# zjkang/Relation-DETR

Hardware: AMD Instinct MI355X
Metric: images/sec @ 800×1333, 300 queries, R50 4-level; achieved HBM GB/s (higher is better)
Workload: dtype bf16; 1 GPU; relation_detr_resnet50_800_1333 transformer stack from feature pyramids: 6 encoder layers (MSDA self-attn, S=22323, 4 levels) + two-stage top-k + 6 decoder layers (relation-biased self-attn + MSDA cross-attn + box refinement) + top-300 detections; backbone/neck excluded; batch_per_gpu=4, global_batch=4, queries=900, levels=4, launch=hipGraph replay, streams=2, gemm_tuning=False, parallelism=image-parallel x1

## Files before the change

### include/relation_detr_amd.h

```cpp
#ifndef RELATION_DETR_AMD_H
#define RELATION_DETR_AMD_H

#include <stdint.h>

#ifdef __cplusplus
extern "C" {
#endif

#define RDETR_ABI_VERSION 3

typedef enum rdetr_status {
    RDETR_OK = 0,
    RDETR_ERR_INVALID_ARG = -1,
    RDETR_ERR_UNSUPPORTED = -2,
    RDETR_ERR_LAUNCH = -3
} rdetr_status;

int rdetr_abi_version(void);
const char *rdetr_status_string(int status);

int rdetr_msda_forward_f32(const float *value, const int64_t *spatial_shapes, const int64_t *level_start_index,
                           const float *sampling_loc, const float *attn_weight, int B, int S, int H, int D,
                           int L, int Nq, int P, float *out, void *stream);

// ... 144 lines not shown
int rdetr_add_layernorm_strided_f32(const float *x, const float *residual, const float *gamma, const float *beta,
                                    long long rows, int C, long long ldx, long long ldr, long long ldo, float eps,
                                    float *out, void *stream);
int rdetr_add_layernorm_strided_bf16(const uint16_t *x, const uint16_t *residual, const uint16_t *gamma,
                                     const uint16_t *beta, long long rows, int C, long long ldx, long long ldr,
                                     long long ldo, float eps, uint16_t *out, void *stream);

int rdetr_add_layernorm_pos_f32(const float *x, const float *residual, const float *gamma, const float *beta,
                                const float *pos, long long rows, int C, long long ldx, long long ldr, long long ldo,
                                long long ldp, long long ldo2, float eps, float *out, float *out2, void *stream);
int rdetr_add_layernorm_pos_bf16(const uint16_t *x, const uint16_t *residual, const uint16_t *gamma,
                                 const uint16_t *beta, const uint16_t *pos, long long rows, int C, long long ldx,
                                 long long ldr, long long ldo, long long ldp, long long ldo2, float eps, uint16_t *out,
                                 uint16_t *out2, void *stream);

int rdetr_box_refine_f32(const void *delta, int delta_is_bf16, const float *ref, long long n, float eps, float *out,
                         void *stream);
int rdetr_sine_pos_embed(const float *pos, long long rows, int n, int F, float temperature, float scale, void *out,
                         int out_is_bf16, void *stream);

int rdetr_zero_masked_rows(void *x, const unsigned char *mask, long long rows, int row_bytes, long long ld_bytes,
                           void *stream);
int rdetr_row_max(const void *x, int is_bf16, long long rows, int C, long long ldx, void *out, void *stream);

long long rdetr_topk_workspace_bytes(int rows, int n, int k);
int rdetr_topk(const void *x, int is_bf16, int rows, int n, int k, void *workspace, float *values, long long *indices, void *stream);

int rdetr_box_head_k256_bf16(const uint16_t *xa, long long lda, const uint16_t *xb, long long ldb, const uint16_t *pw1,
                             const uint16_t *b1, const uint16_t *pw2, const uint16_t *b2, const uint16_t *w3, const uint16_t *b3,
                             const float *reference, int reference_is_logit, float eps, long long M, float *out_a, float *out_b,
                             void *stream);

int rdetr_query_pos_k256_bf16(const uint16_t *emb, long long lde, const uint16_t *query, long long ldq, const uint16_t *pw1a,
                              const uint16_t *pw1b, const uint16_t *b1, const uint16_t *pw2, const uint16_t *b2, const uint16_t *pv1,
                              const uint16_t *c1, const uint16_t *pv2, const uint16_t *c2, long long M, uint16_t *out_pos,
                              uint16_t *out_qpp, void *stream);

int rdetr_encoder_proj_k256_bf16(const uint16_t *x, long long ldx, const uint16_t *xq, long long ldq, const uint16_t *pwv,
                                 const uint16_t *bv, const uint16_t *pwq, const uint16_t *bq, const uint8_t *row_mask, int B, int S,
                                 int q_cols, uint16_t *out_hm, uint16_t *out_q, void *stream);

int rdetr_detections_from_topk(const float *score, const long long *index, const float *boxes, const long long *image_sizes, int B,
                               int N, int C, int K, float *out, void *stream);

int rdetr_scaled_pos(const void *a, const void *scale, const void *query, long long n, int is_bf16, void *pos, void *qp, void *stream);

int rdetr_decoder_reference(const float *reference, const float *valid_ratios, int B, int N, int L, int F, float temperature,
                            float scale, float *ref_in, void *emb, int emb_is_bf16, void *stream);

int rdetr_pyramid_points(const unsigned char *const *level_masks, const int *level_hw, int L, int B, const unsigned char *pad_mask,
                         int keep_is_bf16, float *valid_ratios, float *reference, float *logit, void *keep, void *stream);
int rdetr_nchw_to_tokens(const void *src, const void *add_vec, int is_bf16, int B, int C, int P,
                         long long out_image_stride, long long ld_out, void *out, void *stream);

int rdetr_linear_k256_bf16(const uint16_t *x, long long ldx, const uint16_t *w, const uint16_t *bias, long long M, int N,
                           int relu, uint16_t *out, long long ldo, void *stream);

int rdetr_linear_pack_k256_bf16(const uint16_t *w, uint16_t *packed, void *stream);
int rdetr_linear_ln_k256_bf16(const uint16_t *x, long long ldx, const uint16_t *packed, const uint16_t *bias,
                              const uint16_t *residual, long long ldr, const uint16_t *gamma, const uint16_t *beta, float eps,
                              long long M, uint16_t *out, long long ldo, void *stream);

int rdetr_ffn_k256_pack_bf16(const uint16_t *w1, const uint16_t *w2, int F, uint16_t *packed, void *stream);
int rdetr_ffn_k256_bf16(const uint16_t *x, long long ldx, const uint16_t *packed, const uint16_t *b1, const uint16_t *b2,
                        long long M, int F, uint16_t *out, long long ldo, void *stream);
int rdetr_ffn_ln_k256_bf16(const uint16_t *x, long long ldx, const uint16_t *packed, const uint16_t *b1, const uint16_t *b2,
                           const uint16_t *gamma, const uint16_t *beta, float eps, const uint16_t *pos, long long ldp,
                           long long M, int F, uint16_t *out, long long ldo, uint16_t *out2, long long ldo2, void *stream);
int rdetr_ffn_k256_train_bf16(const uint16_t *x, long long ldx, const uint16_t *packed, const uint16_t *b1, const uint16_t *b2,
                              long long M, int F, uint16_t *out, long long ldo, uint16_t *hid, long long ldh, void *stream);
int rdetr_ffn_k256_backward_bf16(const uint16_t *dy, long long lddy, const uint16_t *packed_t, const uint16_t *hid, long long ldh,
                                 long long M, int F, uint16_t *dh, long long ldd, uint16_t *dx, long long lddx, void *stream);

#ifdef __cplusplus
}
#endif
#endif
```

### relation_detr_amd/_lib.py

```python
from __future__ import annotations

import ctypes
import os

_HERE = os.path.dirname(os.path.abspath(__file__))
LIB_PATH = os.environ.get("RDETR_LIB_PATH") or os.path.join(_HERE, "librelation_detr_amd.so")

_c_int, _c_float, _vp, _c_ll = ctypes.c_int, ctypes.c_float, ctypes.c_void_p, ctypes.c_longlong

SIGNATURES = {
    "rdetr_abi_version": [],
    "rdetr_status_string": [_c_int],
    "rdetr_msda_fast_path": [_c_int] * 4,
    "rdetr_msda_levels_window_ok": [_vp, _vp, _c_int, _c_ll],
    "rdetr_msda_forward_f32": [_vp] * 5 + [_c_int] * 7 + [_vp, _vp],
    "rdetr_msda_forward_bf16": [_vp] * 5 + [_c_int] * 7 + [_vp, _vp],
    "rdetr_msda_forward_fused_f32": [_vp] * 6 + [_c_int] * 8 + [_vp, _vp],
    "rdetr_msda_forward_fused_bf16": [_vp] * 6 + [_c_int] * 8 + [_vp, _vp],
    "rdetr_msda_forward_fused_ex_f32": [_vp] * 4 + [_c_int, _vp, _c_int, _vp, _c_int, _vp] + [_c_int] * 7 + [_vp, _vp],
    "rdetr_msda_forward_fused_ex_bf16": [_vp] * 4 + [_c_int, _vp, _c_int, _vp, _c_int, _vp] + [_c_int] * 7 + [_vp, _vp],
    "rdetr_msda_forward_opt_bf16": [_vp, _c_int] + [_vp] * 4 + [_c_int] * 8 + [_vp, _vp],
    "rdetr_msda_forward_sweep_bf16": [_vp, _c_int] + [_vp] * 4 + [_c_int] * 7 + [_vp, _vp],
    "rdetr_msda_forward_resident_bf16": [_vp] * 5 + [_c_int] * 7 + [_vp, _vp],
    "rdetr_msda_forward_fused_resident_bf16": [_vp, _vp, _vp, _vp, _c_int, _vp, _c_int, _vp, _c_int] + [_c_int] * 7 + [_vp, _vp],
    "rdetr_msda_forward_fused_opt_bf16": [_vp, _c_int, _vp, _vp, _vp, _c_int, _vp, _c_int, _vp, _c_int, _vp] + [_c_int] * 8 + [_vp, _vp],
    "rdetr_msda_forward_fused_strided_bf16": [_vp, _c_ll, _vp, _vp, _vp, _c_int, _vp, _c_int, _vp, _c_int, _vp] + [_c_int] * 7 + [_vp, _vp],
    "rdetr_value_to_head_major_bf16": [_vp, _c_ll, _vp] + [_c_int] * 4 + [_vp, _vp],
    "rdetr_msda_backward_f32": [_vp] * 6 + [_c_int] * 7 + [_vp] * 4,
    "rdetr_msda_backward_det_workspace_bytes": [_c_int] * 7,
    "rdetr_msda_backward_det_f32": [_vp] * 6 + [_c_int] * 7 + [_vp, _c_ll] + [_vp] * 4,
    "rdetr_msda_backward_fused_f32": [_vp] * 6 + [_c_int, _vp] + [_c_int] * 7 + [_vp, _c_ll] + [_vp] * 5,
    "rdetr_msda_backward_fused_bf16": [_vp] * 6 + [_c_int, _vp] + [_c_int] * 7 + [_vp, _c_ll] + [_vp] * 5,
    "rdetr_relation_bias_f32": [_vp] * 4 + [_c_int] * 5 + [_c_float] * 3 + [_vp, _vp],
    "rdetr_relation_bias_ws_f32": [_vp] * 4 + [_c_int] * 5 + [_c_float] * 3 + [_vp, _vp, _vp],
    "rdetr_relation_bias_backward_workspace_bytes": [_c_int] * 3,
    "rdetr_relation_bias_backward_f32": [_vp] * 4 + [_c_int] * 5 + [_c_float] * 3 + [_vp] * 4,
    "rdetr_bias_softmax_f32": [_vp] * 3 + [_c_int] * 3 + [_vp],
    "rdetr_relation_attention_bf16": [_vp] * 3 + [_c_int] * 3 + [_vp, _vp] + [_c_int] * 5 + [_c_float, _vp, _c_int, _vp],
    "rdetr_relation_attention_train_bf16": [_vp] * 3 + [_c_int] * 3 + [_vp, _vp] + [_c_int] * 5 + [_c_float, _vp, _c_int, _vp, _vp],
    "rdetr_relation_attention_backward_workspace_bytes": [_c_int] * 3,
    "rdetr_relation_attention_backward_bf16": [_vp] * 3 + [_c_int] * 3 + [_vp, _c_int, _vp, _vp, _c_int, _vp, _vp] + [_c_int] * 5
                                              + [_c_float, _vp, _c_ll] + [_vp, _c_int] * 3 + [_vp, _vp],
    "rdetr_relation_attention_boxes_bf16": [_vp] * 3 + [_c_int] * 3 + [_vp] * 5 + [_c_int] * 6 + [_c_float] * 4 + [_vp, _c_int, _vp],
    "rdetr_relation_attention_boxes_train_bf16": [_vp] * 3 + [_c_int] * 3 + [_vp] * 5 + [_c_int] * 6 + [_c_float] * 4
                                                 + [_vp, _c_int, _vp, _vp],
    "rdetr_relation_attention_boxes_backward_workspace_bytes": [_c_int] * 4,
    "rdetr_relation_attention_boxes_backward_bf16": [_vp] * 3 + [_c_int] * 3 + [_vp, _c_int, _vp, _vp, _c_int] + [_vp] * 5 + [_c_int] * 6
                                                    + [_c_float] * 4 + [_vp, _c_ll] + [_vp, _c_int] * 3 + [_vp, _vp, _vp],
    "rdetr_box_refine_f32": [_vp, _c_int, _vp, _c_ll, _c_float, _vp, _vp],
    "rdetr_sine_pos_embed": [_vp, _c_ll, _c_int, _c_int, _c_float, _c_float, _vp, _c_int, _vp],
    "rdetr_zero_masked_rows": [_vp, _vp, _c_ll, _c_int, _c_ll, _vp],
    "rdetr_row_max": [_vp, _c_int, _c_ll, _c_int, _c_ll, _vp, _vp],
    "rdetr_topk_workspace_bytes": [_c_int, _c_int, _c_int],
    "rdetr_topk": [_vp, _c_int, _c_int, _c_int, _c_int, _vp, _vp, _vp, _vp],
    "rdetr_box_head_k256_bf16": [_vp, _c_ll, _vp, _c_ll, _vp, _vp, _vp, _vp, _vp, _vp, _vp, _c_int, _c_float, _c_ll, _vp, _vp, _vp],
    "rdetr_query_pos_k256_bf16": [_vp, _c_ll, _vp, _c_ll] + [_vp] * 9 + [_c_ll, _vp, _vp, _vp],
    "rdetr_encoder_proj_k256_bf16": [_vp, _c_ll, _vp, _c_ll] + [_vp] * 5 + [_c_int, _c_int, _c_int, _vp, _vp, _vp],
    "rdetr_detections_from_topk": [_vp, _vp, _vp, _vp, _c_int, _c_int, _c_int, _c_int, _vp, _vp],
    "rdetr_scaled_pos": [_vp, _vp, _vp, _c_ll, _c_int, _vp, _vp, _vp],
    "rdetr_decoder_reference": [_vp, _vp, _c_int, _c_int, _c_int, _c_int, _c_float, _c_float, _vp, _vp, _c_int, _vp],
    "rdetr_pyramid_points": [_vp, _vp, _c_int, _c_int, _vp, _c_int, _vp, _vp, _vp, _vp, _vp],
    "rdetr_linear_k256_bf16": [_vp, _c_ll, _vp, _vp, _c_ll, _c_int, _c_int, _vp, _c_ll, _vp],
    "rdetr_linear_k256_hm_bf16": [_vp, _c_ll, _vp, _vp, _vp, _c_int, _c_int, _vp, _vp],
    "rdetr_linear_pack_k256_bf16": [_vp, _vp, _vp],
    "rdetr_linear_ln_k256_bf16": [_vp, _c_ll, _vp, _vp, _vp, _c_ll, _vp, _vp, _c_float, _c_ll, _vp, _c_ll, _vp],
    "rdetr_ffn_k256_pack_bf16": [_vp, _vp, _c_int, _vp, _vp],
    "rdetr_ffn_k256_bf16": [_vp, _c_ll, _vp, _vp, _vp, _c_ll, _c_int, _vp, _c_ll, _vp],
    "rdetr_ffn_ln_k256_bf16": [_vp, _c_ll, _vp, _vp, _vp, _vp, _vp, _c_float, _vp, _c_ll, _c_ll, _c_int, _vp, _c_ll, _vp, _c_ll, _vp],
    "rdetr_ffn_k256_train_bf16": [_vp, _c_ll, _vp, _vp, _vp, _c_ll, _c_int, _vp, _c_ll, _vp, _c_ll, _vp],
    "rdetr_ffn_k256_backward_bf16": [_vp, _c_ll, _vp, _vp, _c_ll, _c_ll, _c_int, _vp, _c_ll, _vp, _c_ll, _vp],
    "rdetr_nchw_to_tokens": [_vp, _vp, _c_int, _c_int, _c_int, _c_int, _c_ll, _c_ll, _vp, _vp],
    "rdetr_add_layernorm_f32": [_vp] * 4 + [_c_ll, _c_int, _c_float, _vp, _vp],
    "rdetr_add_layernorm_bf16": [_vp] * 4 + [_c_ll, _c_int, _c_float, _vp, _vp],
    "rdetr_add_layernorm_strided_f32": [_vp] * 4 + [_c_ll, _c_int, _c_ll, _c_ll, _c_ll, _c_float, _vp, _vp],
    "rdetr_add_layernorm_strided_bf16": [_vp] * 4 + [_c_ll, _c_int, _c_ll, _c_ll, _c_ll, _c_float, _vp, _vp],
    "rdetr_add_layernorm_pos_f32": [_vp] * 5 + [_c_ll, _c_int] + [_c_ll] * 5 + [_c_float, _vp, _vp, _vp],
    "rdetr_add_layernorm_pos_bf16": [_vp] * 5 + [_c_ll, _c_int] + [_c_ll] * 5 + [_c_float, _vp, _vp, _vp],
}

ERR_INVALID_ARG, ERR_UNSUPPORTED, ERR_LAUNCH = -1, -2, -3

_lib = None


class RdetrError(RuntimeError):
    pass


def load() -> ctypes.CDLL:
    global _lib
    if _lib is not None:
        return _lib
    if not os.path.exists(LIB_PATH):
        raise RdetrError(
            f"{LIB_PATH} not found: the HIP kernels are not built. Run `make -C relation_detr_amd/csrc` "
            "(needs hipcc, --offload-arch=gfx950). There is no CPU or PyTorch fallback for this path.")
    lib = ctypes.CDLL(LIB_PATH)
    for name, argtypes in SIGNATURES.items():
        fn = getattr(lib, name)
        fn.argtypes = argtypes
        fn.restype = ctypes.c_char_p if name == "rdetr_status_string" else (_c_ll if name.endswith("_workspace_bytes") else _c_int)
    if lib.rdetr_abi_version() != 3:
        raise RdetrError(f"ABI version mismatch: library {lib.rdetr_abi_version()}, binding 3")
    _lib = lib
    return lib


def check(status: int, what: str) -> None:
    if status != 0:
        msg = load().rdetr_status_string(status).decode()
        raise RdetrError(f"{what} failed: {msg} (status {status})")
```

### relation_detr_amd/csrc/glue.hip

```cpp
#include "common.h"

namespace rdetr {

template <typename TD> __device__ __forceinline__ float glue_load(const TD *p);
template <> __device__ __forceinline__ float glue_load<float>(const float *p) { return *p; }
template <> __device__ __forceinline__ float glue_load<uint16_t>(const uint16_t *p) { return bf16_bits_to_f32(*p); }

template <typename TD>
__global__ __launch_bounds__(256) void box_refine_kernel(const TD *__restrict__ delta, const float *__restrict__ ref, long long n,
                                                         float eps, float *__restrict__ out)
{
    const long long i = (long long)blockIdx.x * blockDim.x + threadIdx.x;
    if (i >= n) return;
    float x = ref[i];
    x = fminf(fmaxf(x, 0.f), 1.f);
    if (ref[i] != ref[i]) x = ref[i];
    const float x1 = fmaxf(x, eps), x2 = fmaxf(1.f - x, eps);
    const float z = glue_load<TD>(delta + i) + logf(x1 / x2);
    out[i] = 1.f / (1.f + expf(-z));
}

template <typename TO> __device__ __forceinline__ void glue_store(TO *p, float v);
template <> __device__ __forceinline__ void glue_store<float>(float *p, float v) { *p = v; }
template <> __device__ __forceinline__ void glue_store<uint16_t>(uint16_t *p, float v) { *p = (uint16_t)f32_to_bf16_bits(v); }
// ... 124 lines not shown
    const T *s = src + ((size_t)b * C + c0) * (size_t)P + p0;
#pragma unroll 4
    for (int i = ty; i < 64; i += 4)
        tile[i][tx] = (c0 + i < C && p0 + tx < P) ? glue_load<T>(s + (size_t)i * P + tx) : 0.f;
    __syncthreads();
    const float av = (add_vec && c0 + tx < C) ? glue_load<T>(add_vec + c0 + tx) : 0.f;
    T *o = out + (size_t)b * out_image_stride + (size_t)p0 * ld_out + c0;
#pragma unroll 4
    for (int i = ty; i < 64; i += 4)
        if (p0 + i < P && c0 + tx < C) {
            glue_store<T>(o + (size_t)i * ld_out + tx, tile[tx][i] + av);
        }
}

__global__ __launch_bounds__(256) void nchw_to_tokens_bf16_vec_kernel(const uint16_t *__restrict__ src, const uint16_t *__restrict__ add_vec,
                                                                      int C, int P, long long out_image_stride, long long ld_out,
                                                                      uint16_t *__restrict__ out)
{
    __shared__ __attribute__((aligned(16))) uint16_t tile[64][72];
    const int b = blockIdx.z, c0 = blockIdx.y * 64, p0 = blockIdx.x * 64, tid = threadIdx.x;
#pragma unroll
    for (int k = 0; k < 2; ++k) {
        const int it = tid + 256 * k, ch = it >> 3, pg = it & 7;
        u32x4 v = {0u, 0u, 0u, 0u};
        if (c0 + ch < C && p0 + 8 * pg < P)
            v = *reinterpret_cast<const u32x4 *>(src + ((size_t)b * C + c0 + ch) * (size_t)P + p0 + 8 * pg);
        const unsigned w[4] = {v.x, v.y, v.z, v.w};
#pragma unroll
        for (int j = 0; j < 4; ++j) {
            tile[8 * pg + 2 * j][ch] = (uint16_t)(w[j] & 0xffffu);
            tile[8 * pg + 2 * j + 1][ch] = (uint16_t)(w[j] >> 16);
        }
    }
    __syncthreads();
#pragma unroll
    for (int k = 0; k < 2; ++k) {
        const int it = tid + 256 * k, px = it >> 3, cg = it & 7;
        if (p0 + px >= P || c0 + 8 * cg >= C) continue;
        u32x4 v = *reinterpret_cast<const u32x4 *>(&tile[px][8 * cg]);
        if (add_vec) {
            const u32x4 a = *reinterpret_cast<const u32x4 *>(add_vec + c0 + 8 * cg);
            const unsigned vw[4] = {v.x, v.y, v.z, v.w}, aw[4] = {a.x, a.y, a.z, a.w};
            unsigned o[4];
#pragma unroll
            for (int j = 0; j < 4; ++j)
                o[j] = pack_bf16x2(bf16_bits_to_f32(vw[j] & 0xffffu) + bf16_bits_to_f32(aw[j] & 0xffffu),
                                   bf16_bits_to_f32(vw[j] >> 16) + bf16_bits_to_f32(aw[j] >> 16));
            v = u32x4{o[0], o[1], o[2], o[3]};
        }
        *reinterpret_cast<u32x4 *>(out + (size_t)b * out_image_stride + (size_t)(p0 + px) * ld_out + c0 + 8 * cg) = v;
    }
}

struct PyrLevels {
    const unsigned char *mask[8];
    int h[8], w[8], start[8];
};

__global__ __launch_bounds__(64) void valid_ratios_kernel(PyrLevels lv, int L, float *__restrict__ out)
{
    const int l = blockIdx.x, b = blockIdx.y, lane = threadIdx.x;
    const int h = lv.h[l], w = lv.w[l];
    const unsigned char *m = lv.mask[l] + (size_t)b * h * w;
    int cw = 0, ch = 0;
    for (int x = lane; x < w; x += 64) cw += m[x] == 0;
    for (int y = lane; y < h; y += 64) ch += m[(size_t)y * w] == 0;
#pragma unroll
    for (int o = 32; o >= 1; o >>= 1) {
        cw += __shfl_xor(cw, o, 64);
        ch += __shfl_xor(ch, o, 64);
    }
    if (lane == 0) {
        out[((size_t)b * L + l) * 2 + 0] = (float)cw / (float)w;
        out[((size_t)b * L + l) * 2 + 1] = (float)ch / (float)h;
    }
}

template <typename T>
__global__ __launch_bounds__(256) void pyramid_points_kernel(PyrLevels lv, int L, int S, const float *__restrict__ ratios,
                                                             const unsigned char *__restrict__ pad, float *__restrict__ reference,
                                                             float *__restrict__ logit, T *__restrict__ keep)
{
    const int s = blockIdx.x * 256 + threadIdx.x, b = blockIdx.y;
    if (s >= S) return;
    int l = 0;
    while (l + 1 < L && s >= lv.start[l + 1]) ++l;
    const int w = lv.w[l], h = lv.h[l], idx = s - lv.start[l];
    const int y = idx / w, x = idx - y * w;
    const float *vr = ratios + (size_t)b * L * 2;
    const float fx = ((float)x + 0.5f) / (vr[2 * l] * (float)w), fy = ((float)y + 0.5f) / (vr[2 * l + 1] * (float)h);
    float *r = reference + ((size_t)b * S + s) * L * 2;
    for (int k = 0; k < L; ++k) {
        r[2 * k] = fx * vr[2 * k];
        r[2 * k + 1] = fy * vr[2 * k + 1];
    }
    const float wh = 0.05f * (float)(1 << l);
    const float p[4] = {fx, fy, wh, wh};
    bool ok = !(pad && pad[(size_t)b * S + s]);
#pragma unroll
    for (int k = 0; k < 4; ++k) ok = ok && p[k] > 0.01f && p[k] < 0.99f;
    float *lg = logit + ((size_t)b * S + s) * 4;
#pragma unroll
    for (int k = 0; k < 4; ++k) lg[k] = ok ? logf(p[k] / (1.0f - p[k])) : __builtin_inff();
    glue_store<T>(keep + (size_t)b * S + s, ok ? 1.0f : 0.0f);
}

// ... 129 lines not shown
extern "C" int rdetr_zero_masked_rows(void *x, const unsigned char *mask, long long rows, int row_bytes, long long ld_bytes,
                                      void *stream)
{
    if (rows < 0 || row_bytes <= 0 || ld_bytes < row_bytes) return RDETR_ERR_INVALID_ARG;
    if ((row_bytes & 15) || (ld_bytes & 15)) return RDETR_ERR_UNSUPPORTED;
    if (rows == 0) return RDETR_OK;
    if (!x || !mask || (reinterpret_cast<uintptr_t>(x) & 15)) return RDETR_ERR_INVALID_ARG;
    const long long nblk = (rows + 255) / 256;
    if (nblk > 0x7fffffffll) return RDETR_ERR_UNSUPPORTED;
    hipLaunchKernelGGL(zero_masked_rows_kernel, dim3((unsigned)nblk), dim3(256), 0, static_cast<hipStream_t>(stream),
                       static_cast<unsigned char *>(x), mask, rows, row_bytes, ld_bytes);
    return launch_status();
}

extern "C" int rdetr_row_max(const void *x, int is_bf16, long long rows, int C, long long ldx, void *out, void *stream)
{
    if (rows < 0 || C <= 0 || ldx < C) return RDETR_ERR_INVALID_ARG;
    if (rows == 0) return RDETR_OK;
    if (!x || !out) return RDETR_ERR_INVALID_ARG;
    const long long nblk = (rows + 15) / 16;
    if (nblk > 0x7fffffffll) return RDETR_ERR_UNSUPPORTED;
    hipStream_t st = static_cast<hipStream_t>(stream);
    if (is_bf16)
        hipLaunchKernelGGL((row_max_kernel<uint16_t>), dim3((unsigned)nblk), dim3(256), 0, st, static_cast<const uint16_t *>(x), rows, C,
                           ldx, static_cast<uint16_t *>(out));
    else
        hipLaunchKernelGGL((row_max_kernel<float>), dim3((unsigned)nblk), dim3(256), 0, st, static_cast<const float *>(x), rows, C, ldx,
                           static_cast<float *>(out));
    return launch_status();
}

extern "C" int rdetr_nchw_to_tokens(const void *src, const void *add_vec, int is_bf16, int B, int C, int P,
                                    long long out_image_stride, long long ld_out, void *out, void *stream)
{
    if (B < 0 || C <= 0 || P < 0 || ld_out < C || out_image_stride < 0) return RDETR_ERR_INVALID_ARG;
    if (B == 0 || P == 0) return RDETR_OK;
    if (!src || !out) return RDETR_ERR_INVALID_ARG;
    if (B > 65535 || (C + 63) / 64 > 65535) return RDETR_ERR_UNSUPPORTED;
    const dim3 grid((unsigned)((P + 63) / 64), (unsigned)((C + 63) / 64), (unsigned)B);
    hipStream_t st = static_cast<hipStream_t>(stream);
    auto al16 = [](const void *p) { return reinterpret_cast<uintptr_t>(p) % 16 == 0; };
    if (is_bf16 && P % 8 == 0 && C % 8 == 0 && ld_out % 8 == 0 && out_image_stride % 8 == 0 && al16(src) && al16(out) &&
        (!add_vec || al16(add_vec)))
        hipLaunchKernelGGL(nchw_to_tokens_bf16_vec_kernel, grid, dim3(256), 0, st, static_cast<const uint16_t *>(src),
                           static_cast<const uint16_t *>(add_vec), C, P, out_image_stride, ld_out, static_cast<uint16_t *>(out));
    else if (is_bf16)
        hipLaunchKernelGGL((nchw_to_tokens_kernel<uint16_t>), grid, dim3(256), 0, st, static_cast<const uint16_t *>(src),
                           static_cast<const uint16_t *>(add_vec), C, P, out_image_stride, ld_out, static_cast<uint16_t *>(out));
    else
        hipLaunchKernelGGL((nchw_to_tokens_kernel<float>), grid, dim3(256), 0, st, static_cast<const float *>(src),
                           static_cast<const float *>(add_vec), C, P, out_image_stride, ld_out, static_cast<float *>(out));
    return launch_status();
}
```

### relation_detr_amd/csrc/topk.hip

```cpp
#include "common.h"

namespace rdetr {

constexpr int kTkBins = 4096;
constexpr int kTkItems = 16;
constexpr int kTkBlock = 256;
constexpr int kTkChunk = kTkBlock * kTkItems;

struct TkCtrl {
    unsigned bin, above, out_count, cand_count;
};

__device__ __forceinline__ unsigned tk_key(float v)
{
    const unsigned u = __builtin_bit_cast(unsigned, v);
    if (v != v) return 0xffffffffu;
    return (u & 0x80000000u) ? ~u : (u | 0x80000000u);
}
__device__ __forceinline__ float tk_load(const void *x, int is_bf16, size_t i)
{
    return is_bf16 ? bf16_bits_to_f32(static_cast<const uint16_t *>(x)[i]) : static_cast<const float *>(x)[i];
}
__device__ __forceinline__ float tk_value(unsigned key)
{
    if (key == 0xffffffffu) return __builtin_nanf("");
    return __builtin_bit_cast(float, (key & 0x80000000u) ? (key & 0x7fffffffu) : ~key);
}

__global__ __launch_bounds__(kTkBlock) void topk_hist_kernel(const void *__restrict__ x, int is_bf16, int n, unsigned *__restrict__ hist)
{
    __shared__ unsigned h[kTkBins];
    for (int i = threadIdx.x; i < kTkBins; i += kTkBlock) h[i] = 0;
    __syncthreads();
    const size_t row = (size_t)blockIdx.y * n;
    const int base = blockIdx.x * kTkChunk;
#pragma unroll 4
    for (int j = 0; j < kTkItems; ++j) {
        const int i = base + j * kTkBlock + threadIdx.x;
        if (i < n) atomicAdd(&h[tk_key(tk_load(x, is_bf16, row + i)) >> 20], 1u);
    }
    __syncthreads();
    unsigned *g = hist + ((size_t)blockIdx.y * gridDim.x + blockIdx.x) * kTkBins;
    for (int i = threadIdx.x; i < kTkBins; i += kTkBlock) g[i] = h[i];
}

__global__ __launch_bounds__(1024) void topk_scan_kernel(const unsigned *__restrict__ hist, int chunks, int k, TkCtrl *__restrict__ ctrl)
{
    __shared__ unsigned s[1024];
    const int t = threadIdx.x;
    unsigned c0 = 0, c1 = 0, c2 = 0, c3 = 0;
    for (int ch = 0; ch < chunks; ++ch) {
        const u32x4 v = *reinterpret_cast<const u32x4 *>(hist + ((size_t)blockIdx.x * chunks + ch) * kTkBins + 4 * t);
        c0 += v.x; c1 += v.y; c2 += v.z; c3 += v.w;
    }
    s[t] = c0 + c1 + c2 + c3;
    __syncthreads();
    for (int o = 1; o < 1024; o <<= 1) {
        const unsigned v = t + o < 1024 ? s[t + o] : 0u;
        __syncthreads();
        s[t] += v;
// ... 34 lines not shown
        if (i < n) {
            key[j] = tk_key(tk_load(x, is_bf16, row + i));
            const unsigned bin = key[j] >> 20;
            if (bin > bstar) { fw |= 1u << j; ++nw; }
            else if (bin == bstar) { fc |= 1u << j; ++nc; }
        }
    }
    unsigned pw = nw, pc = nc;
#pragma unroll
    for (int o = 1; o < 64; o <<= 1) {
        const unsigned a = __shfl_up(pw, o, 64), bq = __shfl_up(pc, o, 64);
        if (lane >= o) { pw += a; pc += bq; }
    }
    if (lane == 63) { wave_w[wave] = pw; wave_c[wave] = pc; }
    __syncthreads();
    if (threadIdx.x == 0) {
        unsigned tw = 0, tc = 0;
        for (int i = 0; i < kTkBlock / 64; ++i) {
            const unsigned a = wave_w[i], bq = wave_c[i];
            wave_w[i] = tw; wave_c[i] = tc;
            tw += a; tc += bq;
        }
        base_w = tw ? atomicAdd(&ctrl[r].out_count, tw) : 0u;
        base_c = tc ? atomicAdd(&ctrl[r].cand_count, tc) : 0u;
    }
    __syncthreads();
    unsigned ow = base_w + wave_w[wave] + pw - nw, oc = base_c + wave_c[wave] + pc - nc;
#pragma unroll
    for (int j = 0; j < kTkItems; ++j) {
        const int i = base + j * kTkBlock + threadIdx.x;
        const unsigned long long comp = ((unsigned long long)key[j] << 20) | (unsigned long long)(0xfffffu - (unsigned)i);
        if (fw >> j & 1u) w[ow++] = comp;
        if (fc >> j & 1u) c[oc++] = comp;
    }
}

__device__ __forceinline__ unsigned tk_suffix_exclusive(unsigned v, unsigned *wave_tot, int t)
{
    const int lane = t & 63, wave = t >> 6;
    unsigned incl = v;
#pragma unroll
    for (int o = 1; o < 64; o <<= 1) {
        const unsigned a = __shfl_down(incl, o, 64);
        if (lane + o < 64) incl += a;
    }
    if (lane == 0) wave_tot[wave] = incl;
    __syncthreads();
    unsigned above_waves = 0;
    for (int wv = wave + 1; wv < 16; ++wv) above_waves += wave_tot[wv];
    __syncthreads();
    return incl - v + above_waves;
}

__global__ __launch_bounds__(1024) void topk_finish_kernel(const TkCtrl *__restrict__ ctrl, const unsigned long long *__restrict__ cand, int n,
                                                          unsigned long long *__restrict__ winners, int k, float *__restrict__ values,
                                                          long long *__restrict__ indices)
{
    __shared__ unsigned hist[1024];
    __shared__ unsigned wave_tot[16];
    __shared__ unsigned long long keys[1024];
    __shared__ unsigned sel_bin, sel_above, append;
    const int r = blockIdx.x, t = threadIdx.x;
    const unsigned above = ctrl[r].above, cnt = ctrl[r].cand_count;
    const unsigned long long *c = cand + (size_t)r * n;
    unsigned long long *w = winners + (size_t)r * k;
    unsigned need = (unsigned)k - above;
    unsigned long long prefix = 0, pmask = 0;
    for (int shift = 30; shift >= 0; shift -= 10) {
        hist[t] = 0;
        __syncthreads();
        for (unsigned i = t; i < cnt; i += 1024) {
            const unsigned long long v = c[i];
            if ((v & pmask) == prefix) atomicAdd(&hist[(unsigned)(v >> shift) & 1023u], 1u);
        }
        __syncthreads();
        const unsigned mine = hist[t];
        const unsigned ab = tk_suffix_exclusive(mine, wave_tot, t);
        if (ab < need && ab + mine >= need) {
            sel_bin = (unsigned)t;
            sel_above = ab;
        }
        __syncthreads();
        prefix |= (unsigned long long)sel_bin << shift;
        pmask |= 1023ull << shift;
        need -= sel_above;
        __syncthreads();
    }
    const unsigned long long low40 = (1ull << 40) - 1ull;
    if (t == 0) append = 0;
    __syncthreads();
    for (unsigned i = t; i < cnt; i += 1024) {
        const unsigned long long v = c[i];
        if ((v & low40) >= prefix) w[above + atomicAdd(&append, 1u)] = v;
    }
    __syncthreads();
    unsigned long long mine = t < k ? w[t] : 0ull;
    for (int size = 2; size <= 1024; size <<= 1)
        for (int stride = size >> 1; stride > 0; stride >>= 1) {
            unsigned long long other;
            if (stride >= 64) {
                keys[t] = mine;
                __syncthreads();
                other = keys[t ^ stride];
                __syncthreads();
            } else {
                const unsigned lo = __shfl_xor((unsigned)mine, stride, 64), hi = __shfl_xor((unsigned)(mine >> 32), stride, 64);
                other = ((unsigned long long)hi << 32) | lo;
            }
            const bool desc = (t & size) == 0, lower = (t & stride) == 0;
            const bool take_max = desc == lower;
            mine = take_max ? (mine > other ? mine : other) : (mine < other ? mine : other);
        }
    if (t < k) {
        values[(size_t)r * k + t] = tk_value((unsigned)(mine >> 20));
        indices[(size_t)r * k + t] = (long long)(0xfffffu - (unsigned)(mine & 0xfffffu));
    }
}

}

using namespace rdetr;

extern "C" long long rdetr_topk_workspace_bytes(int rows, int n, int k)
{
    if (rows < 0 || n < 0 || k < 0) return -1;
    const long long chunks = (n + kTkChunk - 1) / kTkChunk;
    return (long long)rows * (chunks * kTkBins * 4 + 16 + 8ll * n + 8ll * k);
}

extern "C" int rdetr_topk(const void *x, int is_bf16, int rows, int n, int k, void *workspace, float *values, long long *indices, void *stream)
{
    if (rows < 0 || n <= 0 || k <= 0) return RDETR_ERR_INVALID_ARG;
    if (k > n || k > 1024 || n >= (1 << 20) || rows > 65535) return RDETR_ERR_UNSUPPORTED;
    if (rows == 0) return RDETR_OK;
    if (!x || !workspace || !values || !indices) return RDETR_ERR_INVALID_ARG;
    if (reinterpret_cast<uintptr_t>(workspace) % 16) return RDETR_ERR_UNSUPPORTED;
    hipStream_t st = static_cast<hipStream_t>(stream);
    unsigned char *ws = static_cast<unsigned char *>(workspace);
    const int chunks = (n + kTkChunk - 1) / kTkChunk;
    unsigned *hist = reinterpret_cast<unsigned *>(ws);
    TkCtrl *ctrl = reinterpret_cast<TkCtrl *>(ws + (size_t)rows * chunks * kTkBins * 4);
    unsigned long long *cand = reinterpret_cast<unsigned long long *>(ws + (size_t)rows * ((size_t)chunks * kTkBins * 4 + 16));
    unsigned long long *winners = cand + (size_t)rows * n;
    const dim3 grid((unsigned)chunks, (unsigned)rows);
    hipLaunchKernelGGL(topk_hist_kernel, grid, dim3(kTkBlock), 0, st, x, is_bf16, n, hist);
    hipLaunchKernelGGL(topk_scan_kernel, dim3((unsigned)rows), dim3(1024), 0, st, hist, chunks, k, ctrl);
    hipLaunchKernelGGL(topk_partition_kernel, grid, dim3(kTkBlock), 0, st, x, is_bf16, n, ctrl, winners, k, cand);
    hipLaunchKernelGGL(topk_finish_kernel, dim3((unsigned)rows), dim3(1024), 0, st, ctrl, cand, n, winners, k, values, indices);
    return launch_status();
}
```

### relation_detr_amd/ops.py

```python
from __future__ import annotations

import collections
import weakref
from typing import Optional, Tuple

import torch

from . import _lib


_KEEP: "collections.deque" = collections.deque(maxlen=64)


def _cptr(t: torch.Tensor) -> int:
    if t.is_contiguous():
        return t.data_ptr()
    c = t.contiguous()
    _KEEP.append(c)
    return c.data_ptr()


def _stream_ptr(t: torch.Tensor) -> int:
    return torch.cuda.current_stream(t.device).cuda_stream

# ... 1022 lines not shown
                      scale: float = 6.283185307179586, dtype: torch.dtype = torch.float32):
    _require_device(reference_points, valid_ratios)
    if (reference_points.dtype != torch.float32 or valid_ratios.dtype != torch.float32 or reference_points.dim() != 3
            or reference_points.shape[-1] != 4 or valid_ratios.dim() != 3 or valid_ratios.shape[-1] != 2
            or valid_ratios.shape[0] != reference_points.shape[0] or dtype not in (torch.float32, torch.bfloat16)):
        raise _lib.RdetrError("decoder_reference: reference [B,N,4] fp32, valid_ratios [B,L,2] fp32")
    ref, vr = reference_points.contiguous(), valid_ratios.contiguous()
    B, N, _ = ref.shape
    L = vr.shape[1]
    ref_in = torch.empty(B, N, L, 4, dtype=torch.float32, device=ref.device)
    emb = torch.empty(B, N, 4 * num_pos_feats, dtype=dtype, device=ref.device)
    st = _lib.load().rdetr_decoder_reference(ref.data_ptr(), vr.data_ptr(), B, N, L, num_pos_feats, float(temperature), float(scale),
                                             ref_in.data_ptr(), emb.data_ptr(), int(dtype == torch.bfloat16), _stream_ptr(ref))
    _lib.check(st, "rdetr_decoder_reference")
    return ref_in, emb


def pyramid_points(level_masks, pad_mask: Optional[torch.Tensor], keep_dtype: torch.dtype):
    import ctypes
    _require_device(*level_masks, pad_mask)
    L, B = len(level_masks), level_masks[0].shape[0]
    masks = [m.contiguous() for m in level_masks]
    if any(m.dtype != torch.bool or m.dim() != 3 or m.shape[0] != B for m in masks) or keep_dtype not in (torch.float32, torch.bfloat16):
        raise _lib.RdetrError("pyramid_points: bool masks [B, h, w] per level, keep in float32 or bfloat16")
    S = sum(m.shape[1] * m.shape[2] for m in masks)
    dev = masks[0].device
    pad = None
    if pad_mask is not None:
        if tuple(pad_mask.shape) != (B, S) or pad_mask.dtype != torch.bool:
            raise _lib.RdetrError("pyramid_points: pad_mask must be bool [B, S]")
        pad = pad_mask.contiguous()
    ptrs = (ctypes.c_void_p * L)(*[m.data_ptr() for m in masks])
    hw = (ctypes.c_int * (2 * L))(*[v for m in masks for v in (m.shape[1], m.shape[2])])
    ratios = torch.empty(B, L, 2, dtype=torch.float32, device=dev)
    reference = torch.empty(B, S, L, 2, dtype=torch.float32, device=dev)
    logit = torch.empty(B, S, 4, dtype=torch.float32, device=dev)
    keep = torch.empty(B, S, dtype=keep_dtype, device=dev)
    st = _lib.load().rdetr_pyramid_points(ptrs, hw, L, B, None if pad is None else pad.data_ptr(), int(keep_dtype == torch.bfloat16),
                                          ratios.data_ptr(), reference.data_ptr(), logit.data_ptr(), keep.data_ptr(), _stream_ptr(ratios))
    _lib.check(st, "rdetr_pyramid_points")
    return ratios, reference, logit, keep


def tokens_from_levels(levels, add_vecs=None, out: Optional[torch.Tensor] = None) -> torch.Tensor:
    x0 = levels[0]
    _require_device(*levels)
    B, C = x0.shape[:2]
    S = sum(x.shape[2] * x.shape[3] for x in levels)
    if out is None:
        out = torch.empty(B, S, C, dtype=x0.dtype, device=x0.device)
    if tuple(out.shape) != (B, S, C) or out.dtype != x0.dtype or out.stride(-1) != 1 or (B > 1 and out.stride(0) < S * out.stride(1)):
        raise _lib.RdetrError("tokens_from_levels: out must be [B, S, C] in the levels' dtype with contiguous channels")
    lib, es, row = _lib.load(), out.element_size(), 0
    for l, x in enumerate(levels):
        if x.shape[:2] != (B, C) or x.dtype != x0.dtype:
            raise _lib.RdetrError("tokens_from_levels: levels must agree in batch, channels and dtype")
        x = x.contiguous()
        vec = None
        if add_vecs is not None:
            vec = add_vecs[l].to(x0.dtype).contiguous()
            if vec.numel() != C:
                raise _lib.RdetrError("tokens_from_levels: add_vecs[l] needs C entries")
        P = x.shape[2] * x.shape[3]
        st = lib.rdetr_nchw_to_tokens(x.data_ptr(), vec.data_ptr() if vec is not None else None, int(x0.dtype == torch.bfloat16),
                                      B, C, P, out.stride(0), out.stride(1), out.data_ptr() + row * out.stride(1) * es,
                                      _stream_ptr(x0))
        _lib.check(st, "rdetr_nchw_to_tokens")
        row += P
    return out


def linear_k256_supported(x: torch.Tensor, weight: torch.Tensor) -> bool:
    if not (x.is_cuda and x.dtype == torch.bfloat16 and weight.dtype == torch.bfloat16 and x.shape[-1] == 256
            and weight.dim() == 2 and weight.shape[1] == 256 and weight.shape[0] % 32 == 0 and weight.is_contiguous()):
        return False
    try:
        _, _, ld = _rows_view(x, "linear_k256")
    except _lib.RdetrError:
        return False
    return ld % 8 == 0 and x.data_ptr() % 16 == 0 and weight.data_ptr() % 16 == 0


def linear_k256(x: torch.Tensor, weight: torch.Tensor, bias: Optional[torch.Tensor] = None, relu: bool = False,
                out: Optional[torch.Tensor] = None) -> torch.Tensor:
    _require_device(x, weight, bias, out)
    if not linear_k256_supported(x, weight):
        raise _lib.RdetrError("linear_k256: needs bf16, K = 256, N % 32 == 0, evenly strided 16-byte aligned rows")
    rows, _, ldx = _rows_view(x, "linear_k256")
    N = weight.shape[0]
    if bias is not None and (bias.dtype != torch.bfloat16 or bias.numel() != N):
        raise _lib.RdetrError("linear_k256: bias must be bf16 [N]")
    if out is None:
        out = torch.empty(*x.shape[:-1], N, dtype=x.dtype, device=x.device)
    elif tuple(out.shape) != (*x.shape[:-1], N) or out.dtype != x.dtype:
        raise _lib.RdetrError("linear_k256: out must be [..., N] bf16")
    orows, _, ldo = _rows_view(out, "linear_k256")
    if orows != rows or ldo % 8 or out.data_ptr() % 16:
        raise _lib.RdetrError("linear_k256: out rows must be 16-byte aligned")
    st = _lib.load().rdetr_linear_k256_bf16(x.data_ptr(), ldx, weight.data_ptr(), None if bias is None else _cptr(bias),
                                            rows, N, int(relu), out.data_ptr(), ldo, _stream_ptr(x))
    _lib.check(st, "rdetr_linear_k256_bf16")
    return out


def value_proj_head_major(x: torch.Tensor, weight: torch.Tensor, bias: Optional[torch.Tensor],
                          key_padding_mask: Optional[torch.Tensor] = None) -> torch.Tensor:
    _require_device(x, weight, bias, key_padding_mask)
    if x.dim() != 3 or not linear_k256_supported(x, weight) or tuple(weight.shape) != (256, 256):
        raise _lib.RdetrError("value_proj_head_major: needs bf16 x [B, S, 256] with evenly strided 16-byte aligned rows and a [256, 256] weight")
    B, S, _ = x.shape
    _, _, ldx = _rows_view(x, "value_proj_head_major")
    if bias is not None and (bias.dtype != torch.bfloat16 or bias.numel() != 256):
        raise _lib.RdetrError("value_proj_head_major: bias must be bf16 [256]")
    mask_ptr = None
    if key_padding_mask is not None:
# ... 162 lines not shown
```

Measured before the change: 1052 images/s.

## Fuse per-level NCHW-to-token launches and add single-launch row top-k

Folds the per-level NCHW-to-token transposes into one launch that covers all pyramid levels, with 16-byte vectorized bf16 loads and stores. Adds a single-kernel top-k path for rows of up to 32768 elements. It builds the histogram, finds the boundary bin, partitions candidates and does the refine sort in one 1024-thread block per row, replacing four launches. The goal is to cut launch count and intermediate workspace traffic, at the cost of only one block per row, which limits parallelism when rows are few.

```diff
diff --git a/include/relation_detr_amd.h b/include/relation_detr_amd.h
--- a/include/relation_detr_amd.h
+++ b/include/relation_detr_amd.h
@@ -220,6 +220,8 @@
                          int keep_is_bf16, float *valid_ratios, float *reference, float *logit, void *keep, void *stream);
 int rdetr_nchw_to_tokens(const void *src, const void *add_vec, int is_bf16, int B, int C, int P,
                          long long out_image_stride, long long ld_out, void *out, void *stream);
+int rdetr_nchw_levels_to_tokens(const void *const *level_src, const void *const *level_vec, const int *level_pixels, int L,
+                                int is_bf16, int B, int C, long long out_image_stride, long long ld_out, void *out, void *stream);
 
 int rdetr_linear_k256_bf16(const uint16_t *x, long long ldx, const uint16_t *w, const uint16_t *bias, long long M, int N,
                            int relu, uint16_t *out, long long ldo, void *stream);
diff --git a/relation_detr_amd/_lib.py b/relation_detr_amd/_lib.py
--- a/relation_detr_amd/_lib.py
+++ b/relation_detr_amd/_lib.py
@@ -70,6 +70,7 @@
     "rdetr_ffn_k256_train_bf16": [_vp, _c_ll, _vp, _vp, _vp, _c_ll, _c_int, _vp, _c_ll, _vp, _c_ll, _vp],
     "rdetr_ffn_k256_backward_bf16": [_vp, _c_ll, _vp, _vp, _c_ll, _c_ll, _c_int, _vp, _c_ll, _vp, _c_ll, _vp],
     "rdetr_nchw_to_tokens": [_vp, _vp, _c_int, _c_int, _c_int, _c_int, _c_ll, _c_ll, _vp, _vp],
+    "rdetr_nchw_levels_to_tokens": [_vp, _vp, _vp, _c_int, _c_int, _c_int, _c_int, _c_ll, _c_ll, _vp, _vp],
     "rdetr_add_layernorm_f32": [_vp] * 4 + [_c_ll, _c_int, _c_float, _vp, _vp],
     "rdetr_add_layernorm_bf16": [_vp] * 4 + [_c_ll, _c_int, _c_float, _vp, _vp],
     "rdetr_add_layernorm_strided_f32": [_vp] * 4 + [_c_ll, _c_int, _c_ll, _c_ll, _c_ll, _c_float, _vp, _vp],
diff --git a/relation_detr_amd/csrc/glue.hip b/relation_detr_amd/csrc/glue.hip
--- a/relation_detr_amd/csrc/glue.hip
+++ b/relation_detr_amd/csrc/glue.hip
@@ -200,6 +200,83 @@
     }
 }
 
+struct TokLevels {
+    const void *src[8];
+    const void *vec[8];
+    int pixels[8], row0[8];
+    int tile0[9];
+};
+
+template <typename T>
+__global__ __launch_bounds__(256) void nchw_levels_to_tokens_kernel(TokLevels lv, int L, int C, long long out_image_stride,
+                                                                    long long ld_out, int wide, T *__restrict__ out)
+{
+    int l = 0;
+    while (l + 1 < L && (int)blockIdx.x >= lv.tile0[l + 1]) ++l;
+    const int P = lv.pixels[l], p0 = ((int)blockIdx.x - lv.tile0[l]) * 64;
+    const int b = blockIdx.z, c0 = blockIdx.y * 64, tid = threadIdx.x;
+    const int tx = tid & 63, ty = tid >> 6;
+    const T *src = static_cast<const T *>(lv.src[l]) + ((size_t)b * C + c0) * (size_t)P + p0;
+    const T *add_vec = static_cast<const T *>(lv.vec[l]);
+    T *o = out + (size_t)b * out_image_stride + ((size_t)lv.row0[l] + p0) * ld_out + c0;
+    if constexpr (sizeof(T) == 4) {
+        __shared__ float tile[64][65];
+#pragma unroll 4
+        for (int i = ty; i < 64; i += 4) tile[i][tx] = (c0 + i < C && p0 + tx < P) ? src[(size_t)i * P + tx] : 0.f;
+        __syncthreads();
+        const float av = (add_vec && c0 + tx < C) ? add_vec[c0 + tx] : 0.f;
+#pragma unroll 4
+        for (int i = ty; i < 64; i += 4)
+            if (p0 + i < P && c0 + tx < C) o[(size_t)i * ld_out + tx] = tile[tx][i] + av;
+    } else {
+        __shared__ __attribute__((aligned(16))) uint16_t tile[64][72];
+        if (P % 8 == 0 && reinterpret_cast<uintptr_t>(lv.src[l]) % 16 == 0) {
+#pragma unroll
+            for (int k = 0; k < 2; ++k) {
+                const int it = tid + 256 * k, ch = it >> 3, pg = it & 7;
+                u32x4 v = {0u, 0u, 0u, 0u};
+                if (c0 + ch < C && p0 + 8 * pg < P) v = *reinterpret_cast<const u32x4 *>(src + (size_t)ch * P + 8 * pg);
+                const unsigned w[4] = {v.x, v.y, v.z, v.w};
+#pragma unroll
+                for (int j = 0; j < 4; ++j) {
+                    tile[8 * pg + 2 * j][ch] = (uint16_t)(w[j] & 0xffffu);
+                    tile[8 * pg + 2 * j + 1][ch] = (uint16_t)(w[j] >> 16);
+                }
+            }
+        } else {
+#pragma unroll 4
+            for (int i = ty; i < 64; i += 4)
+                tile[tx][i] = (c0 + i < C && p0 + tx < P) ? src[(size_t)i * P + tx] : (uint16_t)0;
+        }
+        __syncthreads();
+        if (wide) {
+#pragma unroll
+            for (int k = 0; k < 2; ++k) {
+                const int it = tid + 256 * k, px = it >> 3, cg = it & 7;
+                if (p0 + px >= P || c0 + 8 * cg >= C) continue;
+                u32x4 v = *reinterpret_cast<const u32x4 *>(&tile[px][8 * cg]);
+                if (add_vec) {
+                    const u32x4 a = *reinterpret_cast<const u32x4 *>(add_vec + c0 + 8 * cg);
+                    const unsigned vw[4] = {v.x, v.y, v.z, v.w}, aw[4] = {a.x, a.y, a.z, a.w};
+                    unsigned s[4];
+#pragma unroll
+                    for (int j = 0; j < 4; ++j)
+                        s[j] = pack_bf16x2(bf16_bits_to_f32(vw[j] & 0xffffu) + bf16_bits_to_f32(aw[j] & 0xffffu),
+                                           bf16_bits_to_f32(vw[j] >> 16) + bf16_bits_to_f32(aw[j] >> 16));
+                    v = u32x4{s[0], s[1], s[2], s[3]};
+                }
+                *reinterpret_cast<u32x4 *>(o + (size_t)px * ld_out + 8 * cg) = v;
+            }
+        } else {
+            const float av = (add_vec && c0 + tx < C) ? bf16_bits_to_f32(add_vec[c0 + tx]) : 0.f;
+#pragma unroll 4
+            for (int i = ty; i < 64; i += 4)
+                if (p0 + i < P && c0 + tx < C)
+                    o[(size_t)i * ld_out + tx] = (uint16_t)f32_to_bf16_bits(bf16_bits_to_f32(tile[i][tx]) + av);
+        }
+    }
+}
+
 struct PyrLevels {
     const unsigned char *mask[8];
     int h[8], w[8], start[8];
@@ -435,3 +512,39 @@
                            static_cast<const float *>(add_vec), C, P, out_image_stride, ld_out, static_cast<float *>(out));
     return launch_status();
 }
+
+extern "C" int rdetr_nchw_levels_to_tokens(const void *const *level_src, const void *const *level_vec, const int *level_pixels, int L,
+                                           int is_bf16, int B, int C, long long out_image_stride, long long ld_out, void *out,
+                                           void *stream)
+{
+    if (L <= 0 || B < 0 || C <= 0 || !level_src || !level_pixels || ld_out < C || out_image_stride < 0) return RDETR_ERR_INVALID_ARG;
+    if (L > 8 || B > 65535 || (C + 63) / 64 > 65535 || (is_bf16 != 0 && is_bf16 != 1)) return RDETR_ERR_UNSUPPORTED;
+    auto al16 = [](const void *p) { return reinterpret_cast<uintptr_t>(p) % 16 == 0; };
+    TokLevels lv = {};
+    long long rows = 0, tiles = 0;
+    bool wide = C % 8 == 0 && ld_out % 8 == 0 && out_image_stride % 8 == 0 && al16(out);
+    for (int l = 0; l < L; ++l) {
+        if (level_pixels[l] < 0 || (level_pixels[l] > 0 && !level_src[l])) return RDETR_ERR_INVALID_ARG;
+        lv.src[l] = level_src[l];
+        lv.vec[l] = level_vec ? level_vec[l] : nullptr;
+        lv.pixels[l] = level_pixels[l];
+        lv.row0[l] = (int)rows;
+        lv.tile0[l] = (int)tiles;
+        rows += level_pixels[l];
+        tiles += (level_pixels[l] + 63) / 64;
+        if (rows >= (1ll << 31)) return RDETR_ERR_UNSUPPORTED;
+        wide = wide && al16(lv.vec[l]);
+    }
+    lv.tile0[L] = (int)tiles;
+    if (B == 0 || tiles == 0) return RDETR_OK;
+    if (!out) return RDETR_ERR_INVALID_ARG;
+    const dim3 grid((unsigned)tiles, (unsigned)((C + 63) / 64), (unsigned)B);
+    hipStream_t st = static_cast<hipStream_t>(stream);
+    if (is_bf16)
+        hipLaunchKernelGGL((nchw_levels_to_tokens_kernel<uint16_t>), grid, dim3(256), 0, st, lv, L, C, out_image_stride, ld_out,
+                           (int)wide, static_cast<uint16_t *>(out));
+    else
+        hipLaunchKernelGGL((nchw_levels_to_tokens_kernel<float>), grid, dim3(256), 0, st, lv, L, C, out_image_stride, ld_out, 0,
+                           static_cast<float *>(out));
+    return launch_status();
+}
diff --git a/relation_detr_amd/csrc/topk.hip b/relation_detr_amd/csrc/topk.hip
--- a/relation_detr_amd/csrc/topk.hip
+++ b/relation_detr_amd/csrc/topk.hip
@@ -6,6 +6,7 @@
 constexpr int kTkItems = 16;
 constexpr int kTkBlock = 256;
 constexpr int kTkChunk = kTkBlock * kTkItems;
+constexpr int kTkOneLaunchMaxN = 32768;
 
 struct TkCtrl {
     unsigned bin, above, out_count, cand_count;
@@ -146,18 +147,12 @@
     return incl - v + above_waves;
 }
 
-__global__ __launch_bounds__(1024) void topk_finish_kernel(const TkCtrl *__restrict__ ctrl, const unsigned long long *__restrict__ cand, int n,
-                                                          unsigned long long *__restrict__ winners, int k, float *__restrict__ values,
-                                                          long long *__restrict__ indices)
-{
-    __shared__ unsigned hist[1024];
-    __shared__ unsigned wave_tot[16];
-    __shared__ unsigned long long keys[1024];
-    __shared__ unsigned sel_bin, sel_above, append;
-    const int r = blockIdx.x, t = threadIdx.x;
-    const unsigned above = ctrl[r].above, cnt = ctrl[r].cand_count;
-    const unsigned long long *c = cand + (size_t)r * n;
-    unsigned long long *w = winners + (size_t)r * k;
+__device__ __forceinline__ void tk_refine_sort(unsigned above, unsigned cnt, const unsigned long long *c, unsigned long long *w, int k, int r,
+                                               unsigned *hist, unsigned *wave_tot, unsigned long long *keys, unsigned *sel,
+                                               float *__restrict__ values, long long *__restrict__ indices)
+{
+    unsigned &sel_bin = sel[0], &sel_above = sel[1], &append = sel[2];
+    const int t = threadIdx.x;
     unsigned need = (unsigned)k - above;
     unsigned long long prefix = 0, pmask = 0;
     for (int shift = 30; shift >= 0; shift -= 10) {
@@ -211,6 +206,152 @@
     }
 }
 
+__global__ __launch_bounds__(1024) void topk_finish_kernel(const TkCtrl *__restrict__ ctrl, const unsigned long long *__restrict__ cand, int n,
+                                                          unsigned long long *__restrict__ winners, int k, float *__restrict__ values,
+                                                          long long *__restrict__ indices)
+{
+    __shared__ unsigned hist[1024];
+    __shared__ unsigned wave_tot[16];
+    __shared__ unsigned long long keys[1024];
+    __shared__ unsigned sel[3];
+    const int r = blockIdx.x;
+    tk_refine_sort(ctrl[r].above, ctrl[r].cand_count, cand + (size_t)r * n, winners + (size_t)r * k, k, r, hist, wave_tot, keys, sel, values,
+                   indices);
+}
+
+constexpr int kTkUnroll = 4;
+
+template <bool BF16> __device__ __forceinline__ void tk_vec_keys(const u32x4 v, unsigned *key)
+{
+    const unsigned w[4] = {v.x, v.y, v.z, v.w};
+#pragma unroll
+    for (int j = 0; j < 4; ++j) {
+        if (BF16) {
+            key[2 * j] = tk_key(bf16_bits_to_f32(w[j] & 0xffffu));
+            key[2 * j + 1] = tk_key(bf16_bits_to_f32(w[j] >> 16));
+        } else {
+            key[j] = tk_key(__builtin_bit_cast(float, w[j]));
+        }
+    }
+}
+
+template <bool BF16>
+__global__ __launch_bounds__(1024) void topk_row_kernel(const void *__restrict__ x, int n, int k, unsigned long long *__restrict__ cand,
+                                                        unsigned long long *__restrict__ winners, float *__restrict__ values,
+                                                        long long *__restrict__ indices)
+{
+    constexpr int kPer = BF16 ? 8 : 4, kEs = BF16 ? 2 : 4;
+    __shared__ unsigned hist[kTkBins];
+    __shared__ unsigned wave_tot[16];
+    __shared__ unsigned long long keys[1024];
+    __shared__ unsigned sel[3], bnd[2], cls[2];
+    const int r = blockIdx.x, t = threadIdx.x, lane = t & 63;
+    const unsigned char *row = static_cast<const unsigned char *>(x) + (size_t)r * n * kEs;
+    unsigned long long *c = cand + (size_t)r * n, *w = winners + (size_t)r * k;
+    const int head = min(n, (int)(((16u - (unsigned)(reinterpret_cast<uintptr_t>(row) & 15u)) & 15u) / kEs));
+    const int nv = (n - head) / kPer, tail0 = head + nv * kPer;
+    const u32x4 *vrow = reinterpret_cast<const u32x4 *>(row + (size_t)head * kEs);
+    auto edge_index = [&](int e) { return e < head ? e : tail0 + (e - head); };
+    const int edges = head + n - tail0;
+    for (int i = t; i < kTkBins; i += 1024) hist[i] = 0;
+    if (t == 0) cls[0] = cls[1] = 0;
+    __syncthreads();
+    for (int v0 = t; v0 < nv; v0 += 1024 * kTkUnroll) {
+        u32x4 d[kTkUnroll] = {};
+#pragma unroll
+        for (int u = 0; u < kTkUnroll; ++u)
+            if (v0 + 1024 * u < nv) d[u] = vrow[v0 + 1024 * u];
+#pragma unroll
+        for (int u = 0; u < kTkUnroll; ++u)
+            if (v0 + 1024 * u < nv) {
+                unsigned key[kPer];
+                tk_vec_keys<BF16>(d[u], key);
+                unsigned bin = key[0] >> 20, run = 1;
+#pragma unroll
+                for (int j = 1; j < kPer; ++j) {
+                    const unsigned bj = key[j] >> 20;
+                    if (bj != bin) {
+                        atomicAdd(&hist[bin], run);
+                        bin = bj;
+                        run = 0;
+                    }
+                    ++run;
+                }
+                atomicAdd(&hist[bin], run);
+            }
+    }
+    if (t < edges) atomicAdd(&hist[tk_key(tk_load(row, BF16, (size_t)edge_index(t))) >> 20], 1u);
+    __syncthreads();
+    {
+        const unsigned cb[4] = {hist[4 * t], hist[4 * t + 1], hist[4 * t + 2], hist[4 * t + 3]};
+        unsigned run = tk_suffix_exclusive(cb[0] + cb[1] + cb[2] + cb[3], wave_tot, t);
+#pragma unroll
+        for (int j = 3; j >= 0; --j) {
+            if (run < (unsigned)k && run + cb[j] >= (unsigned)k) {
+                bnd[0] = (unsigned)(4 * t + j);
+                bnd[1] = run;
+            }
+            run += cb[j];
+        }
+    }
+    __syncthreads();
+    const unsigned bstar = bnd[0], above = bnd[1];
+    for (int v0 = t; v0 - t < nv; v0 += 1024 * kTkUnroll) {
+        u32x4 d[kTkUnroll] = {};
+#pragma unroll
+        for (int u = 0; u < kTkUnroll; ++u)
+            if (v0 + 1024 * u < nv) d[u] = vrow[v0 + 1024 * u];
+        unsigned key[kTkUnroll * kPer];
+        unsigned nw = 0, nc = 0, fw = 0, fc = 0;
+#pragma unroll
+        for (int u = 0; u < kTkUnroll; ++u)
+            if (v0 + 1024 * u < nv) {
+                tk_vec_keys<BF16>(d[u], key + u * kPer);
+#pragma unroll
+                for (int j = 0; j < kPer; ++j) {
+                    const unsigned bin = key[u * kPer + j] >> 20;
+                    if (bin > bstar) { fw |= 1u << (u * kPer + j); ++nw; }
+                    else if (bin == bstar) { fc |= 1u << (u * kPer + j); ++nc; }
+                }
+            }
+        if (__ballot((nw | nc) != 0) == 0ull) continue;
+        unsigned pw = nw, pc = nc;
+#pragma unroll
+        for (int o = 1; o < 64; o <<= 1) {
+            const unsigned a = __shfl_up(pw, o, 64), bq = __shfl_up(pc, o, 64);
+            if (lane >= o) { pw += a; pc += bq; }
+        }
+        unsigned bw = 0, bc = 0;
+        if (lane == 63) {
+            bw = pw ? atomicAdd(&cls[0], pw) : 0u;
+            bc = pc ? atomicAdd(&cls[1], pc) : 0u;
+        }
+        unsigned ow = __shfl(bw, 63, 64) + pw - nw, oc = __shfl(bc, 63, 64) + pc - nc;
+#pragma unroll
+        for (int u = 0; u < kTkUnroll; ++u)
+#pragma unroll
+            for (int j = 0; j < kPer; ++j) {
+                const int q = u * kPer + j;
+                if ((fw | fc) >> q & 1u) {
+                    const unsigned i = (unsigned)(head + (v0 + 1024 * u) * kPer + j);
+                    const unsigned long long comp = ((unsigned long long)key[q] << 20) | (unsigned long long)(0xfffffu - i);
+                    if (fw >> q & 1u) w[ow++] = comp;
+                    else c[oc++] = comp;
+                }
+            }
+    }
+    if (t < edges) {
+        const unsigned i = (unsigned)edge_index(t);
+        const unsigned key1 = tk_key(tk_load(row, BF16, (size_t)i));
+        const unsigned long long comp = ((unsigned long long)key1 << 20) | (unsigned long long)(0xfffffu - i);
+        if ((key1 >> 20) > bstar) w[atomicAdd(&cls[0], 1u)] = comp;
+        else if ((key1 >> 20) == bstar) c[atomicAdd(&cls[1], 1u)] = comp;
+    }
+    __threadfence_block();
+    __syncthreads();
+    tk_refine_sort(above, cls[1], c, w, k, r, hist, wave_tot, keys, sel, values, indices);
+}
+
 }
 
 using namespace rdetr;
@@ -236,6 +377,13 @@
     TkCtrl *ctrl = reinterpret_cast<TkCtrl *>(ws + (size_t)rows * chunks * kTkBins * 4);
     unsigned long long *cand = reinterpret_cast<unsigned long long *>(ws + (size_t)rows * ((size_t)chunks * kTkBins * 4 + 16));
     unsigned long long *winners = cand + (size_t)rows * n;
+    if (n <= kTkOneLaunchMaxN && reinterpret_cast<uintptr_t>(x) % (is_bf16 ? 2 : 4) == 0) {
+        if (is_bf16)
+            hipLaunchKernelGGL((topk_row_kernel<true>), dim3((unsigned)rows), dim3(1024), 0, st, x, n, k, cand, winners, values, indices);
+        else
+            hipLaunchKernelGGL((topk_row_kernel<false>), dim3((unsigned)rows), dim3(1024), 0, st, x, n, k, cand, winners, values, indices);
+        return launch_status();
+    }
     const dim3 grid((unsigned)chunks, (unsigned)rows);
     hipLaunchKernelGGL(topk_hist_kernel, grid, dim3(kTkBlock), 0, st, x, is_bf16, n, hist);
     hipLaunchKernelGGL(topk_scan_kernel, dim3((unsigned)rows), dim3(1024), 0, st, hist, chunks, k, ctrl);
diff --git a/relation_detr_amd/ops.py b/relation_detr_amd/ops.py
--- a/relation_detr_amd/ops.py
+++ b/relation_detr_amd/ops.py
@@ -1098,15 +1098,28 @@
     if tuple(out.shape) != (B, S, C) or out.dtype != x0.dtype or out.stride(-1) != 1 or (B > 1 and out.stride(0) < S * out.stride(1)):
         raise _lib.RdetrError("tokens_from_levels: out must be [B, S, C] in the levels' dtype with contiguous channels")
     lib, es, row = _lib.load(), out.element_size(), 0
+    xs, vecs = [], []
     for l, x in enumerate(levels):
         if x.shape[:2] != (B, C) or x.dtype != x0.dtype:
             raise _lib.RdetrError("tokens_from_levels: levels must agree in batch, channels and dtype")
-        x = x.contiguous()
+        xs.append(x.contiguous())
         vec = None
         if add_vecs is not None:
             vec = add_vecs[l].to(x0.dtype).contiguous()
             if vec.numel() != C:
                 raise _lib.RdetrError("tokens_from_levels: add_vecs[l] needs C entries")
+        vecs.append(vec)
+    L = len(xs)
+    if L <= 8:
+        import ctypes
+        src = (ctypes.c_void_p * L)(*[x.data_ptr() for x in xs])
+        vp = (ctypes.c_void_p * L)(*[None if v is None else v.data_ptr() for v in vecs])
+        pix = (ctypes.c_int * L)(*[x.shape[2] * x.shape[3] for x in xs])
+        st = lib.rdetr_nchw_levels_to_tokens(src, vp, pix, L, int(x0.dtype == torch.bfloat16), B, C, out.stride(0), out.stride(1),
+                                             out.data_ptr(), _stream_ptr(x0))
+        _lib.check(st, "rdetr_nchw_levels_to_tokens")
+        return out
+    for x, vec in zip(xs, vecs):
         P = x.shape[2] * x.shape[3]
         st = lib.rdetr_nchw_to_tokens(x.data_ptr(), vec.data_ptr() if vec is not None else None, int(x0.dtype == torch.bfloat16),
                                       B, C, P, out.stride(0), out.stride(1), out.data_ptr() + row * out.stride(1) * es,
```

After: 1068 images/s, median of 6. 1.6% higher.
